# PlanNoa/video_super_resolution

Measured on NVIDIA B200. Metric: sr_frames_per_s_4x_1080p_out, higher is better.
Workload: dtype bf16

## Files before the change

include/vsr_b200.h:

```cpp
#ifndef VSR_B200_H_
#define VSR_B200_H_

#include <stddef.h>
#include <stdint.h>

#ifdef __cplusplus
extern "C" {
#endif

#define VSR_OK 0
#define VSR_ERR_INVALID_ARG 1
#define VSR_ERR_UNSUPPORTED 2
#define VSR_ERR_WORKSPACE 3
#define VSR_ERR_STATE 4
#define VSR_ERR_CUDA_BASE 1000

typedef void* vsr_stream_t;

const char* vsr_version(void);
uint64_t vsr_launch_count(void);
void vsr_launch_count_reset(void);
const char* vsr_error_string(int code);

int vsr_resample2d_forward(const float* input1, const float* flow, float* output,
// ... 156 lines not shown
int vsr_srfbn_profile_launches(vsr_srfbn_plan* plan, float* ms, int32_t* kclass, int32_t capacity);

int vsr_srfbn_debug_premix(const vsr_srfbn_plan* plan, float* out_maps, vsr_stream_t stream);

int vsr_test_pointwise(const void* x_bf16, int64_t rows, int K, const float* w_host,
                       const float* b_host, float slope, int act, void* y_bf16,
                       void* workspace, size_t workspace_bytes, vsr_stream_t stream);
int vsr_test_deconv(const void* x_bf16, int B, int h, int w, const float* w_host,
                    const float* b_host, float slope, int block_layout, void* y_bf16,
                    void* workspace, size_t workspace_bytes, vsr_stream_t stream);
int vsr_test_x2_layer(const void* x_bf16, int up, int B, int h, int w, const float* w_host,
                      const float* b_host, float slope, void* y_bf16, void* workspace,
                      size_t workspace_bytes, vsr_stream_t stream);
size_t vsr_test_workspace_bytes(int B, int h, int w);
int vsr_test_fused_down(const void* hr_bf16, int nsrc, int B, int h, int w, const float* wt_host,
                        const float* bt_host, float slope_t, const float* wd_host, const float* bd_host,
                        float slope_d, void* y_bf16, void* workspace, size_t workspace_bytes,
                        vsr_stream_t stream);
int vsr_test_fused_updown(const void* lr_bf16, void* hr_bf16, int nsrc, int store, int B, int h, int w,
                          const float* wu_host, const float* bu_host, float slope_u, const float* wt_host,
                          const float* bt_host, float slope_t, const float* wd_host, const float* bd_host,
                          float slope_d, void* y_bf16, void* workspace, size_t workspace_bytes,
                          vsr_stream_t stream);

#ifdef __cplusplus
}
#endif
#endif
```

video_super_resolution_b200/_lib.py:

```python
from __future__ import annotations

import ctypes
import os

_HERE = os.path.dirname(os.path.abspath(__file__))
LIB_PATH = os.path.join(_HERE, "libvsr_b200.so")

c_void_p = ctypes.c_void_p
c_int = ctypes.c_int
c_i64 = ctypes.c_int64
c_size_t = ctypes.c_size_t
c_float = ctypes.c_float


class VsrError(RuntimeError):
    pass


class SrfbnConfig(ctypes.Structure):
    _fields_ = [("num_maps", ctypes.c_int32), ("h", ctypes.c_int32), ("w", ctypes.c_int32),
                ("num_steps", ctypes.c_int32), ("num_groups", ctypes.c_int32),
                ("num_features", ctypes.c_int32), ("upscale", ctypes.c_int32)]


# ... 60 lines not shown
    "vsr_srfbn_forward": (c_int, [c_void_p, c_void_p, c_void_p, c_void_p]),
    "vsr_srfbn_forward_u8": (c_int, [c_void_p, c_void_p, c_void_p, c_void_p, c_void_p]),
    "vsr_srfbn_prepare_refresh": (c_int, [c_void_p, c_int]),
    "vsr_srfbn_forward_refresh_u8": (c_int, [c_void_p, c_void_p, c_void_p, c_void_p, c_int, c_void_p]),
    "vsr_srfbn_plan_set_map_range": (c_int, [c_void_p, c_int, c_int]),
    "vsr_srfbn_forward_maps": (c_int, [c_void_p, c_void_p, c_void_p]),
    "vsr_srfbn_forward_maps_refresh": (c_int, [c_void_p, c_void_p, c_int, c_void_p]),
    "vsr_srfbn_pack_bands": (c_int, [c_void_p, ctypes.POINTER(c_int), c_int, c_void_p, c_void_p]),
    "vsr_srfbn_fuse_band": (c_int, [c_void_p, c_void_p, c_int, c_void_p, c_void_p, c_void_p]),
    "vsr_unpack_bands": (c_int, [c_void_p, c_void_p, c_int, c_i64, c_i64, ctypes.POINTER(c_int), c_int, c_i64,
                                 c_void_p]),
    "vsr_srfbn_kernel_class_name":(ctypes.c_char_p, [c_int]),
    "vsr_srfbn_profile_enable": (c_int, [c_void_p, c_int]),
    "vsr_srfbn_profile_read": (c_int, [c_void_p, c_void_p, c_void_p, c_void_p, c_void_p]),
    "vsr_srfbn_profile_launches": (c_int, [c_void_p, c_void_p, c_void_p, c_int]),
    "vsr_srfbn_debug_premix": (c_int, [c_void_p, c_void_p, c_void_p]),
    "vsr_test_pointwise": (c_int, [c_void_p, c_i64, c_int, c_void_p, c_void_p, c_float, c_int, c_void_p, c_void_p, c_size_t, c_void_p]),
    "vsr_test_deconv": (c_int, [c_void_p, c_int, c_int, c_int, c_void_p, c_void_p, c_float, c_int, c_void_p, c_void_p, c_size_t, c_void_p]),
    "vsr_test_fused_down": (c_int, [c_void_p, c_int, c_int, c_int, c_int, c_void_p, c_void_p, c_float, c_void_p, c_void_p,
                                    c_float, c_void_p, c_void_p, c_size_t, c_void_p]),
    "vsr_test_fused_updown": (c_int, [c_void_p, c_void_p, c_int, c_int, c_int, c_int, c_int, c_void_p, c_void_p, c_float,
                                      c_void_p, c_void_p, c_float, c_void_p, c_void_p, c_float, c_void_p, c_void_p,
                                      c_size_t, c_void_p]),
    "vsr_test_x2_layer": (c_int, [c_void_p, c_int, c_int, c_int, c_int, c_void_p, c_void_p, c_float, c_void_p, c_void_p, c_size_t, c_void_p]),
    "vsr_test_workspace_bytes": (c_size_t, [c_int, c_int, c_int]),
}

_lib = None


def lib():
    global _lib
    if _lib is None:
        if not os.path.exists(LIB_PATH):
            raise ImportError(
                f"{LIB_PATH} is missing: build it with `python -m video_super_resolution_b200.build` "
                "(nvcc, sm_100a).  This package has no CPU or PyTorch fallback.")
        L = ctypes.CDLL(LIB_PATH)
        for name, (res, args) in SIGNATURES.items():
            fn = getattr(L, name)
            fn.restype = res
            fn.argtypes = args
        _lib = L
    return _lib


# ... 13 lines not shown
```

video_super_resolution_b200/csrc/fused_down.cuh:

```cuda
#pragma once
#include "igemm.cuh"

namespace vsr {

constexpr int kFusedEpiWarps = 16;
constexpr int kFusedWdWarp = 2 + kFusedEpiWarps;
constexpr int kFusedBWarp = kFusedWdWarp + 1;
constexpr int kFusedThreads = 32 * (kFusedBWarp + 1);
constexpr int kFusedMaxStages = 16;
constexpr int kWdGroupBytes = 128 * 128 * 2;
constexpr int kWdRingBytes = 2 * kWdGroupBytes;
constexpr int kWtChunkBytes = 32 * 32 * 2;
constexpr int kHBytes = 128 * 128 * 2;
constexpr int kXchgBytes = 3 * 4 * 16 * 8 * 4;
constexpr int kLRBox = 16 * 9 * 64;
constexpr int kLRBytes = 2 * kLRBox;
constexpr int kWuTapBytes = 128 * 32 * 2;

struct alignas(64) FusedDownParams {
  CUtensorMap hr_maps[kMaxSources];
  CUtensorMap h0_map;
  CUtensorMap wt_map;
  CUtensorMap wd_map;
  int32_t nsrc;
// ... 4 lines not shown
  const float* down_bias;
  float* part;
  void* lr_out;
  CUtensorMap up_map;
  CUtensorMap wu_map;
  const float* up_bias;
  int32_t hr_store;
};

__device__ __forceinline__ void tmem_ld8(uint32_t taddr, uint32_t (&v)[8]) {
  asm volatile("tcgen05.ld.sync.aligned.32x32b.x8.b32 {%0, %1, %2, %3, %4, %5, %6, %7}, [%8];"
               : "=r"(v[0]), "=r"(v[1]), "=r"(v[2]), "=r"(v[3]), "=r"(v[4]), "=r"(v[5]), "=r"(v[6]), "=r"(v[7])
               : "r"(taddr)
               : "memory");
}

template <bool HAS_TRAN>
inline size_t fused_down_smem_bytes(int nsrc, int num_stages) {
  size_t wt = HAS_TRAN ? ((size_t)nsrc * kWtChunkBytes + 1023) / 1024 * 1024 : 0;
  size_t stage = HAS_TRAN ? 16384 : 2 * 16384;
  return 1024 + kWdRingBytes + wt + (HAS_TRAN ? kHBytes : 0) + (size_t)num_stages * stage + 1024 + kXchgBytes;
}

inline size_t fused_updown_smem_bytes(int nsrc, int num_stages) {
  return fused_down_smem_bytes<true>(nsrc, num_stages) + kLRBytes;
}

template <bool HAS_TRAN, bool MERGED>
__device__ __forceinline__ void fused_down_body(const FusedDownParams& p) {
  static_assert(HAS_TRAN || !MERGED, "the merged kernel needs phase A");
  constexpr int kStageBytes = HAS_TRAN ? 16384 : 2 * 16384;
  constexpr int kTmemCols = HAS_TRAN ? 512 : 256;
  constexpr uint32_t kDB = MERGED ? 384 : HAS_TRAN ? 256 : 0;
  constexpr int kDBToggle = MERGED ? 0 : 1;
  constexpr uint32_t kTU = 256;

  extern __shared__ uint8_t smem_raw[];
  uint8_t* smem = smem_raw + ((1024u - (smem_u32(smem_raw) & 1023u)) & 1023u);
  uint8_t* s_wd = smem;
  uint8_t* s_wt = s_wd + kWdRingBytes;
  const int wt_region = HAS_TRAN ? ((p.nsrc * kWtChunkBytes + 1023) / 1024 * 1024) : 0;
  uint8_t* s_h = s_wt + wt_region;
  uint8_t* s_lr = s_h + (HAS_TRAN ? kHBytes : 0);
  uint8_t* s_a = s_lr + (MERGED ? kLRBytes : 0);
  uint8_t* tail = s_a + p.num_stages * kStageBytes;
  uint64_t* full_bar = reinterpret_cast<uint64_t*>(tail);
  uint64_t* empty_bar = full_bar + kFusedMaxStages;
  uint64_t* w_full = empty_bar + kFusedMaxStages;
  uint64_t* wd_full = w_full + 1;
  uint64_t* wd_empty = wd_full + 2;
  uint64_t* da_full = wd_empty + 2;
  uint64_t* da_empty = da_full + 2;
  uint64_t* h_full = da_empty + 2;
  uint64_t* h_empty = h_full + 1;
  uint64_t* db_full = h_empty + 1;
  uint64_t* db_empty = db_full + 2;
  uint32_t* tmem_ptr = reinterpret_cast<uint32_t*>(db_empty + 2);
  uint64_t* tu_full = db_empty + 3;
  uint64_t* tu_empty = tu_full + 1;
  uint64_t* u_full = tu_empty + 1;
  uint64_t* lr_full = u_full + 1;
  uint64_t* lr_empty = lr_full + 1;
  float* s_bias = reinterpret_cast<float*>(tail + 512);
  float* s_down = s_bias + 36;
  float* s_ubias = s_down + 36;
  float4* s_x = reinterpret_cast<float4*>(tail + 1024);
// ... 80 lines not shown
                tma_load_4d(s_a + s * kStageBytes + 16384, &p.h0_map, &full_bar[s], 0, x0, y0, b * 8 + 2 * g + 1);
              }
              __syncwarp();
              if (++s == p.num_stages) { s = 0; phase ^= 1; }
            }
          }
        }
      }
    }
  } else if (warp == 1 || (HAS_TRAN && warp == kFusedBWarp)) {
    {
    constexpr uint32_t idesc_a = make_idesc(32);
    constexpr uint32_t idesc_b = make_idesc(128);
    if (HAS_TRAN && warp == 1) mbar_wait(w_full, 0);
    tc_fence_after();
    int s = 0;
    uint32_t phase = 0;
    uint32_t n_a[2] = {0, 0}, n_b[2] = {0, 0}, n_h = 0, n_wd = 0;
    int tb = 0;
    const uint64_t dA = make_smem_desc<128>(smem_u32(s_a));
    const uint64_t dWt = make_smem_desc<64>(smem_u32(s_wt));
    const uint64_t dH = make_smem_desc<128>(smem_u32(s_h));
    const uint64_t dWd = make_smem_desc<128>(smem_u32(s_wd));
    uint32_t n_tu = 0, n_lr = 0, n_u = 0;

    auto issue_u = [&](int g) {
      constexpr uint32_t idesc_u = make_idesc(128);
      const uint64_t dLR = make_smem_desc<64>(smem_u32(s_lr));
      const uint64_t dWu = make_smem_desc<64>(smem_u32(s_wd));
      if (g == 0) mbar_wait(lr_full, n_lr & 1);
      mbar_wait(tu_empty, (n_tu & 1) ^ 1);
      mbar_wait(&wd_full[0], n_tu & 1);
      tc_fence_after();
      if (elect_one()) {
#pragma unroll
        for (int t = 0; t < 4; ++t)
#pragma unroll
          for (int k = 0; k < 2; ++k)
            umma_bf16(tmem_base + kTU, dLR + (uint64_t)(((t & 1) * kLRBox + (t >> 1) * 1024) >> 4) + 2 * k,
                      dWu + (uint64_t)((t * kWuTapBytes) >> 4) + 2 * k, idesc_u, (uint32_t)((t | k) != 0));
        umma_commit(&wd_empty[0]);
        umma_commit(tu_full);
        if (g == 3) umma_commit(lr_empty);
      }
      __syncwarp();
      ++n_tu;
      if (g == 3) ++n_lr;
    };

    auto issue_a = [&](int g) {
      const int buf = g & 1;
      mbar_wait(&da_empty[buf], (n_a[buf] & 1) ^ 1);
      tc_fence_after();
      for (int pair = 0; pair < 2; ++pair)
        for (int j = 0; j < p.nsrc - (MERGED ? 1 : 0); ++j) {
          mbar_wait(&full_bar[s], phase);
          tc_fence_after();
          const uint64_t a0 = dA + (uint64_t)((s * kStageBytes) >> 4);
          const uint64_t b0 = dWt + (uint64_t)((j * kWtChunkBytes) >> 4);
          const uint32_t d0 = tmem_base + (uint32_t)(buf * 128 + pair * 64);
          if (elect_one()) {
            const uint32_t acc = (uint32_t)(j != 0);
            umma_bf16(d0, a0, b0, idesc_a, acc);
            umma_bf16(d0, a0 + 2, b0 + 2, idesc_a, 1u);
            umma_bf16(d0 + 32, a0 + 4, b0, idesc_a, acc);
            umma_bf16(d0 + 32, a0 + 6, b0 + 2, idesc_a, 1u);
            umma_commit(&empty_bar[s]);
            if (!MERGED && pair == 1 && j == p.nsrc - 1) umma_commit(&da_full[buf]);
          }
          __syncwarp();
          if (++s == p.num_stages) { s = 0; phase ^= 1; }
        }
      if (MERGED) {
        mbar_wait(u_full, n_u & 1);
        tc_fence_after();
        const uint64_t b0 = dWt + (uint64_t)(((p.nsrc - 1) * kWtChunkBytes) >> 4);
        if (elect_one()) {
          for (int pair = 0; pair < 2; ++pair) {
            const uint64_t a0 = dH + (uint64_t)((pair * 16384) >> 4);
            const uint32_t d0 = tmem_base + (uint32_t)(buf * 128 + pair * 64);
            umma_bf16(d0, a0, b0, idesc_a, 1u);
            umma_bf16(d0, a0 + 2, b0 + 2, idesc_a, 1u);
            umma_bf16(d0 + 32, a0 + 4, b0, idesc_a, 1u);
            umma_bf16(d0 + 32, a0 + 6, b0 + 2, idesc_a, 1u);
          }
          umma_commit(&da_full[buf]);
        }
        __syncwarp();
        ++n_u;
      }
      ++n_a[buf];
    };
    auto issue_b = [&](int g) {
      uint64_t a0;
      if (HAS_TRAN) {
        mbar_wait(h_full, n_h & 1);
        a0 = dH;
      } else {
        mbar_wait(&full_bar[s], phase);
        a0 = dA + (uint64_t)((s * kStageBytes) >> 4);
      }
      if (g == 0) mbar_wait(&db_empty[tb], (n_b[tb] & 1) ^ 1);
      const int wslot = MERGED ? 1 : (int)(n_wd & 1);
      mbar_wait(&wd_full[wslot], MERGED ? (n_wd & 1) : ((n_wd >> 1) & 1));
      tc_fence_after();
      const uint32_t d = tmem_base + kDB + (uint32_t)(tb * 128);
      const uint64_t b0 = dWd + (uint64_t)((wslot * kWdGroupBytes) >> 4);
      if (elect_one()) {
#pragma unroll
        for (int kc = 0; kc < 2; ++kc)
#pragma unroll
          for (int k = 0; k < 4; ++k)
            umma_bf16(d, a0 + (uint64_t)(kc * 1024 + k * 2), b0 + (uint64_t)(kc * 1024 + k * 2), idesc_b,
                      (uint32_t)((g | kc | k) != 0));
        umma_commit(&wd_empty[wslot]);
        if (HAS_TRAN) umma_commit(h_empty);
        else umma_commit(&empty_bar[s]);
        if (g == 3) umma_commit(&db_full[tb]);
      }
      __syncwarp();
      ++n_wd;
      if (HAS_TRAN) ++n_h;
      else if (++s == p.num_stages) { s = 0; phase ^= 1; }
      if (g == 3) { ++n_b[tb]; tb ^= kDBToggle; }
    };

    for (int tile = cta; tile < total_tiles; tile += ncta) {
      if (HAS_TRAN) {
        if (warp == 1) {
          for (int g = 0; g < 4; ++g) {
            if (MERGED) issue_u(g);
            issue_a(g);
          }
        } else {
          for (int g = 0; g < 4; ++g) issue_b(g);
        }
      } else {
        for (int g = 0; g < 4; ++g) issue_b(g);
      }
    }
    }
  } else if (MERGED && warp == kFusedWdWarp) {
    uint32_t n_wu = 0, n_wdm = 0, n_lrl = 0;
    auto load_u = [&](int tile, int g) {
      if (g == 0) {
        int x0, y0, b;
        tile_coord(tile, x0, y0, b);
        mbar_wait(lr_empty, (n_lrl & 1) ^ 1);
        if (elect_one()) {
          mbar_expect_tx(lr_full, (uint32_t)kLRBytes);
          tma_load_4d(s_lr, &p.up_map, lr_full, 0, x0 - 1, y0 - 1, b);
          tma_load_4d(s_lr + kLRBox, &p.up_map, lr_full, 0, x0, y0 - 1, b);
        }
        __syncwarp();
        ++n_lrl;
// ... 48 lines not shown
      tile_coord(tile, x0, y0, b);
      const int Yb = y0 + (row >> 4), Xb = x0 + (row & 15);
      const bool in_tensor = (Yb <= p.lr_h) && (Xb <= p.lr_w);
      if (HAS_TRAN) {
#pragma unroll 1
        for (int g = 0; g < 4; ++g) {
          const int buf = g & 1;
          if (MERGED) {
            mbar_wait_poll(tu_full, m_u & 1);
            tc_fence_after();
            uint32_t v[32];
            tmem_ld32(lane_base + kTU + (uint32_t)(sub * 32), v);
            tmem_ld_wait();
            tc_fence_before();
            mbar_arrive_warp(tu_empty);
            ++m_u;
            const int s16 = g * 4 + sub, ry = s16 >> 2, rx = s16 & 3;
            const int Yt = 4 * Yb + ry - 2, Xt = 4 * Xb + rx - 2;
            const bool inside = (Yt >= 0) && (Yt < 4 * p.lr_h) && (Xt >= 0) && (Xt < 4 * p.lr_w);
            uint32_t o[16];
            const PreluCfg pcu = make_prelu(s_ubias[32], 1);
            convert32(v, s_ubias, pcu, o);
            if (__builtin_expect(!inside, 0)) zero16(o);
            mbar_wait(h_empty, (m_h & 1) ^ 1);
            uint8_t* urow = s_h + (sub >> 1) * 16384 + row * 128;
#pragma unroll
            for (int j = 0; j < 4; ++j) {
              const int piece = (sub & 1) * 4 + j;
              *reinterpret_cast<uint4*>(urow + ((piece ^ (row & 7)) << 4)) =
                  make_uint4(o[4 * j], o[4 * j + 1], o[4 * j + 2], o[4 * j + 3]);
            }
            fence_async_smem();
            asm volatile("bar.sync 1, %0;" ::"n"(32 * kFusedEpiWarps) : "memory");
            if (threadIdx.x == 64) {
              if (p.hr_store) {
                tma_store_4d(&p.hr_maps[p.nsrc - 1], s_h, 0, x0, y0, b * 8 + 2 * g);
                tma_store_4d(&p.hr_maps[p.nsrc - 1], s_h + 16384, 0, x0, y0, b * 8 + 2 * g + 1);
                tma_store_commit();
              }
              mbar_arrive(u_full);
            }
          }
          mbar_wait_poll(&da_full[buf], m_a[buf] & 1);
          tc_fence_after();
          uint32_t o[16];
          uint32_t v[32];
          tmem_ld32(lane_base + (uint32_t)(buf * 128 + sub * 32), v);
          tmem_ld_wait();
          tc_fence_before();
          mbar_arrive_warp(&da_empty[buf]);
          const int s16 = g * 4 + sub, ry = s16 >> 2, rx = s16 & 3;
          const bool ring = (Yb == 0 && ry < 2) || (Yb == p.lr_h && ry >= 2) || (Xb == 0 && rx < 2) ||
                            (Xb == p.lr_w && rx >= 2);
          convert32(v, s_bias, pc, o);
          if (__builtin_expect(!(in_tensor && !ring), 0)) zero16(o);
          ++m_a[buf];
          if (MERGED) {
            if (p.hr_store) {
              if (threadIdx.x == 64) tma_store_wait_read();
              asm volatile("bar.sync 1, %0;" ::"n"(32 * kFusedEpiWarps) : "memory");
            }
          } else {
            mbar_wait(h_empty, (m_h & 1) ^ 1);
          }
          uint8_t* hrow = s_h + (sub >> 1) * 16384 + (row >> 3) * 1024 + (row & 7) * 128;
#pragma unroll
          for (int j = 0; j < 4; ++j) {
            const int piece = (sub & 1) * 4 + j;
            *reinterpret_cast<uint4*>(hrow + ((piece ^ (row & 7)) << 4)) =
                make_uint4(o[4 * j], o[4 * j + 1], o[4 * j + 2], o[4 * j + 3]);
          }
          fence_async_smem();
          mbar_arrive_warp(h_full);
          ++m_h;
        }
      }
      mbar_wait_poll(&db_full[tb], m_b[tb] & 1);
      tc_fence_after();
      uint32_t v[4][8];
#pragma unroll
// ... 56 lines not shown
          }
        }
      }
      ++m_b[tb];
      tb ^= kDBToggle;
    }
    if (MERGED && threadIdx.x == 64) asm volatile("cp.async.bulk.wait_group 0;" ::: "memory");
  }

  tc_fence_before();
  __syncthreads();
  if (warp == 1) {
    tc_fence_after();
    tmem_dealloc<kTmemCols>(tmem_base);
  }
}

template <bool HAS_TRAN>
__global__ void __launch_bounds__(kFusedThreads, 1)
fused_down_kernel(const __grid_constant__ FusedDownParams p) {
  fused_down_body<HAS_TRAN, false>(p);
}

__global__ void __launch_bounds__(kFusedThreads, 1)
fused_updown_kernel(const __grid_constant__ FusedDownParams p) {
  fused_down_body<true, true>(p);
}

constexpr int kFinalizePeriod = 8;
__global__ void __launch_bounds__(256)
finalize_lr_kernel(const float4* __restrict__ part, const float* __restrict__ bias, uint4* __restrict__ out, int B, int h,
                   int w) {
  constexpr int period = kFinalizePeriod;
  const float slope = __ldg(bias + 32);
  const int R = h / period, Cc = w / 16;
  const int64_t nA = (int64_t)B * R * w, nB = (int64_t)B * (h - R) * Cc;
  const int64_t n8 = (nA + nB) * 4;
  for (int64_t i = (int64_t)blockIdx.x * blockDim.x + threadIdx.x; i < n8; i += (int64_t)gridDim.x * blockDim.x) {
    const int c8 = (int)(i & 3);
    int64_t it = i >> 2;
    int b, Y, X;
    if (it < nA) {
      X = (int)(it % w);
      const int64_t r = it / w;
      Y = (int)(r % R) * period + period - 1;
      b = (int)(r / R);
    } else {
      it -= nA;
      X = (int)(it % Cc) * 16 + 15;
// ... 26 lines not shown
```

video_super_resolution_b200/csrc/srfbn.cu:

```cuda
#include "fused_down.cuh"

#include <string.h>

#include <algorithm>
#include <new>
#include <vector>

namespace vsr {
namespace {

constexpr int kNF = 32;
constexpr int kGroups = 6;
constexpr int kMaxMaps = 64;

typedef CUresult (*EncodeTiledFn)(CUtensorMap*, CUtensorMapDataType, cuuint32_t, void*, const cuuint64_t*,
                                  const cuuint64_t*, const cuuint32_t*, const cuuint32_t*, CUtensorMapInterleave,
                                  CUtensorMapSwizzle, CUtensorMapL2promotion, CUtensorMapFloatOOBfill);

EncodeTiledFn encode_fn() {
  static EncodeTiledFn fn = nullptr;
  if (!fn) {
    void* p = nullptr;
    cudaDriverEntryPointQueryResult q;
    if (cudaGetDriverEntryPoint("cuTensorMapEncodeTiled", &p, cudaEnableDefault, &q) == cudaSuccess &&
// ... 9 lines not shown
  cuuint64_t dims[4] = {(cuuint64_t)C, (cuuint64_t)W, (cuuint64_t)H, (cuuint64_t)B};
  cuuint64_t strides[3] = {(cuuint64_t)C * 2, (cuuint64_t)C * 2 * W, (cuuint64_t)C * 2 * W * H};
  cuuint32_t box[4] = {(cuuint32_t)ck, (cuuint32_t)tw, (cuuint32_t)th, 1};
  cuuint32_t es[4] = {1, 1, 1, 1};
  CUresult r = enc(m, CU_TENSOR_MAP_DATA_TYPE_BFLOAT16, 4, const_cast<void*>(base), dims, strides, box, es,
                   CU_TENSOR_MAP_INTERLEAVE_NONE, ck == 32 ? CU_TENSOR_MAP_SWIZZLE_64B : CU_TENSOR_MAP_SWIZZLE_128B,
                   CU_TENSOR_MAP_L2_PROMOTION_L2_128B, CU_TENSOR_MAP_FLOAT_OOB_FILL_NONE);
  return r == CUDA_SUCCESS ? VSR_OK : VSR_ERR_CUDA_BASE + 999;
}

int make_w_map(CUtensorMap* m, const void* base, int64_t K, int64_t N, int ck, int bn) {
  EncodeTiledFn enc = encode_fn();
  if (!enc) return VSR_ERR_STATE;
  cuuint64_t dims[2] = {(cuuint64_t)K, (cuuint64_t)N};
  cuuint64_t strides[1] = {(cuuint64_t)K * 2};
  cuuint32_t box[2] = {(cuuint32_t)ck, (cuuint32_t)bn};
  cuuint32_t es[2] = {1, 1};
  CUresult r = enc(m, CU_TENSOR_MAP_DATA_TYPE_BFLOAT16, 2, const_cast<void*>(base), dims, strides, box, es,
                   CU_TENSOR_MAP_INTERLEAVE_NONE, ck == 32 ? CU_TENSOR_MAP_SWIZZLE_64B : CU_TENSOR_MAP_SWIZZLE_128B,
                   CU_TENSOR_MAP_L2_PROMOTION_L2_256B, CU_TENSOR_MAP_FLOAT_OOB_FILL_NONE);
  return r == CUDA_SUCCESS ? VSR_OK : VSR_ERR_CUDA_BASE + 999;
}

enum Variant : int { V_PW32 = 0, V_PW128, V_DECONV, V_CONVOUT, V_FUSED_TRAN, V_FUSED_PLAIN, V_FINALIZE, V_DECONV2, V_DOWN2, V_FUSED_UPDOWN, V_COUNT };

static_assert(VSR_SRFBN_KERNEL_CLASSES == 10, "header constant");
enum KClass : int { KC_IM2COL = 0, KC_CONV_IN, KC_PW_LR, KC_PW_HR, KC_DECONV, KC_DOWNCONV, KC_CONV_OUT, KC_FC, KC_FUSED_DOWN, KC_FINALIZE, KC_COUNT };

struct Layer {
  int variant;
  IgemmParams p;
  FusedDownParams f;
  float* fin_acc;
  const float* fin_bias;
  void* fin_out;
  int64_t fin_n8;
  int fin_w, fin_h, fin_b;
  int grid;
  size_t smem;
  int kclass;
  double flops;
  double bytes;
};

template <int MODE, int CK, int BN>
int launch_variant(const Layer& L, cudaStream_t st) {
  static PerDeviceOnce once;
// ... 2 lines not shown
    cudaError_t e = cudaFuncSetAttribute(igemm_kernel<MODE, CK, BN>, cudaFuncAttributeMaxDynamicSharedMemorySize,
                                         227 * 1024);
    if (e != cudaSuccess) return cuda_status(e);
    once.mark(dev);
  }
  igemm_kernel<MODE, CK, BN><<<L.grid, igemm_threads(MODE), L.smem, st>>>(L.p);
  return after_launch();
}

template <bool HAS_TRAN>
int launch_fused(const Layer& L, cudaStream_t st) {
  static PerDeviceOnce once;
  int dev;
  if (once.needed(&dev)) {
    cudaError_t e = cudaFuncSetAttribute(fused_down_kernel<HAS_TRAN>, cudaFuncAttributeMaxDynamicSharedMemorySize,
                                         227 * 1024);
    if (e != cudaSuccess) return cuda_status(e);
    once.mark(dev);
  }
  fused_down_kernel<HAS_TRAN><<<L.grid, kFusedThreads, L.smem, st>>>(L.f);
  return after_launch();
}

int launch_fused_updown(const Layer& L, cudaStream_t st) {
  static PerDeviceOnce once;
  int dev;
  if (once.needed(&dev)) {
    cudaError_t e = cudaFuncSetAttribute(fused_updown_kernel, cudaFuncAttributeMaxDynamicSharedMemorySize, 227 * 1024);
    if (e != cudaSuccess) return cuda_status(e);
    once.mark(dev);
  }
  fused_updown_kernel<<<L.grid, kFusedThreads, L.smem, st>>>(L.f);
  return after_launch();
}

int launch_layer(const Layer& L, cudaStream_t st) {
  switch (L.variant) {
    case V_FUSED_UPDOWN: return launch_fused_updown(L, st);
    case V_FUSED_TRAN: return launch_fused<true>(L, st);
    case V_FUSED_PLAIN: return launch_fused<false>(L, st);
    case V_FINALIZE: {
      const int R = L.fin_h / kFinalizePeriod;
      const int64_t items = ((int64_t)L.fin_b * R * L.fin_w + (int64_t)L.fin_b * (L.fin_h - R) * (L.fin_w / 16)) * 4;
      if (items == 0) return VSR_OK;
      int64_t blocks = ceil_div64(items, 256);
      if (blocks > kNumSMs * 16) blocks = kNumSMs * 16;
      finalize_lr_kernel<<<(int)blocks, 256, 0, st>>>(reinterpret_cast<const float4*>(L.fin_acc), L.fin_bias,
                                                      reinterpret_cast<uint4*>(L.fin_out), L.fin_b, L.fin_h, L.fin_w);
      return after_launch();
    }
    case V_PW32: return launch_variant<EPI_ROWS, 32, 32>(L, st);
    case V_PW128: return launch_variant<EPI_ROWS, 32, 128>(L, st);
    case V_DECONV: return launch_variant<EPI_DECONV, 32, 256>(L, st);
    case V_CONVOUT: return launch_variant<EPI_CONV_OUT, 32, 32>(L, st);
    case V_DECONV2: return launch_variant<EPI_DECONV2, 32, 128>(L, st);
    case V_DOWN2: return launch_variant<EPI_DOWN2, 64, 96>(L, st);
    default: return VSR_ERR_INVALID_ARG;
  }
}

size_t variant_smem(int variant, int chunks, size_t ring) {
// ... 278 lines not shown
  f.num_stages = tran ? 7 : 5;
  f.tiles_x = ceil_div(w + 1, 16);
  f.tiles_y = ceil_div(h + 1, 8);
  f.batch = B;
  f.lr_h = h;
  f.lr_w = w;
  f.tran_bias = tran_bias_dev;
  f.down_bias = down_bias_dev;
  f.part = part;
  f.lr_out = lr_out;
  while (f.num_stages > 2 && (tran ? fused_down_smem_bytes<true>(nsrc, f.num_stages)
                                   : fused_down_smem_bytes<false>(nsrc, f.num_stages)) > 227 * 1024)
    --f.num_stages;
  L.smem = tran ? fused_down_smem_bytes<true>(nsrc, f.num_stages) : fused_down_smem_bytes<false>(nsrc, f.num_stages);
  int64_t total = (int64_t)f.tiles_x * f.tiles_y * B;
  L.grid = (int)(total < kNumSMs ? total : kNumSMs);
  const double lrpx = (double)B * h * w;
  L.kclass = KC_FUSED_DOWN;
  L.flops = lrpx * 131072.0 + (tran ? lrpx * 16.0 * 2.0 * 32.0 * nsrc * 32.0 : 0.0);
  L.bytes = lrpx * 64.0 * (16.0 * nsrc) + lrpx * 64.0;
  return VSR_OK;
}

inline bool updown_merged(int nsrc) { return nsrc >= 4; }

int build_fused_updown(Layer& L, const void* up_in, const void* const* hr, int nsrc, int store, int B, int h, int w,
                       const void* wu_dev, const float* up_bias_dev, const void* wt_dev, const float* tran_bias_dev,
                       const void* wd_dev, const float* down_bias_dev, float* part, void* lr_out) {
  memset(&L, 0, sizeof(L));
  L.variant = V_FUSED_UPDOWN;
  FusedDownParams& f = L.f;
  if (nsrc < 2 || nsrc > kMaxSources || (store && !hr[nsrc - 1])) return VSR_ERR_UNSUPPORTED;
  int rc;
  for (int j = 0; j < nsrc - (store ? 0 : 1); ++j) {
    rc = make_act_map(&f.hr_maps[j], hr[j], 64, w + 1, h + 1, 8 * B, 64, 16, 8);
    if (rc) return rc;
  }
  rc = make_w_map(&f.wt_map, wt_dev, 32 * nsrc, 32, 32, 32);
  if (rc) return rc;
  rc = make_w_map(&f.wd_map, wd_dev, 512, 128, 64, 128);
  if (rc) return rc;
  rc = make_act_map(&f.up_map, up_in, kNF, w, h, B, 32, kTW, kTH + 1);
  if (rc) return rc;
  rc = make_w_map(&f.wu_map, wu_dev, 4 * kNF, 512, 32, 128);
  if (rc) return rc;
  f.nsrc = nsrc;
  f.tiles_x = ceil_div(w + 1, 16);
  f.tiles_y = ceil_div(h + 1, 8);
  f.batch = B;
  f.lr_h = h;
  f.lr_w = w;
  f.tran_bias = tran_bias_dev;
  f.down_bias = down_bias_dev;
  f.up_bias = up_bias_dev;
  f.part = part;
  f.lr_out = lr_out;
  f.hr_store = store;
  const int64_t total = (int64_t)f.tiles_x * f.tiles_y * B;
  L.grid = (int)(total < kNumSMs ? total : kNumSMs);
  f.num_stages = 7;
  while (f.num_stages > 2 && fused_updown_smem_bytes(nsrc, f.num_stages) > 227 * 1024) --f.num_stages;
  L.smem = fused_updown_smem_bytes(nsrc, f.num_stages);
  const double lrpx = (double)B * h * w;
  L.kclass = KC_FUSED_DOWN;
  L.flops = lrpx * 131072.0 * 2.0 + lrpx * 16.0 * 2.0 * 32.0 * nsrc * 32.0;
  L.bytes = lrpx * 64.0 + lrpx * 64.0 * 16.0 * (nsrc - 1 + (store ? 1 : 0)) + lrpx * 64.0;
  return VSR_OK;
}

int build_finalize(Layer& L, float* acc, const float* bias_dev, void* out, int64_t pixels, int h, int w) {
  memset(&L, 0, sizeof(L));
  L.variant = V_FINALIZE;
  L.fin_acc = acc;
  L.fin_bias = bias_dev;
  L.fin_out = out;
  L.fin_n8 = pixels * 4;
  L.fin_w = w;
  L.fin_h = h;
  L.fin_b = (int)(pixels / ((int64_t)h * w));
  L.kclass = KC_FINALIZE;
  L.flops = 0;
  L.bytes = 0;
  return VSR_OK;
}

// ... 299 lines not shown

static int swept_maps(const vsr_srfbn_plan* pl) { return pl->windows * (pl->map1 - pl->map0); }

static bool all_maps(const vsr_srfbn_plan* pl) { return pl->map1 - pl->map0 == pl->cfg.num_maps; }

static void layout_workspace(vsr_srfbn_plan* pl, int chunk, int swept) {
  const vsr_srfbn_config& c = pl->cfg;
  const size_t P = (size_t)chunk * c.h * c.w;
  const size_t Rb = (size_t)chunk * (c.h + 1) * (c.w + 1) * 16;
  size_t off = 0;
  auto put = [&](size_t bytes) {
    size_t o = off;
    off = align_up(off + bytes, 1024);
    return o;
  };
  pl->o_a0 = put(P * 64);
  pl->o_c128 = put(P * 256);
  pl->o_xfeat = put(P * 64);
  pl->o_hidden = put(P * 64);
  for (int i = 0; i < 7; ++i) pl->o_lr[i] = put(P * 64);
  pl->o_u = put(P * 64);
  const size_t s2 = (size_t)c.upscale * c.upscale;
  const bool x2 = c.upscale == 2;
  for (int i = 0; i < 6; ++i) pl->o_hr[i] = put(x2 ? P * s2 * 64 : (i == 5 && updown_merged(6)) ? 0 : Rb * 64);
  pl->o_hb = put(P * s2 * 64);
  pl->o_ht = put(x2 ? P * s2 * 64 : 0);
  pl->o_acc = put(x2 ? 0 : P * 512);
  pl->o_premix = put((size_t)swept * c.h * c.w * s2 * 3 * 4);
  pl->ws_bytes = off;
}

static int set_shape(vsr_srfbn_plan* pl, int windows, int m0, int m1) {
  if (windows > 1 && m1 - m0 != pl->cfg.num_maps) return VSR_ERR_UNSUPPORTED;
  const int swept = windows * (m1 - m0);
  for (int mc = swept; mc >= 1; --mc) {
    if (swept % mc) continue;
    layout_workspace(pl, mc, swept);
    if (pl->ws_cap == 0 || pl->ws_bytes <= pl->ws_cap) {
      pl->windows = windows;
      pl->map0 = m0;
      pl->map1 = m1;
      pl->chunk_maps = mc;
      return VSR_OK;
    }
  }
  layout_workspace(pl, pl->chunk_maps, swept_maps(pl));
  return VSR_ERR_WORKSPACE;
// ... 173 lines not shown
      if (i > 0) {
        Src s[6];
        for (int j = 0; j <= i; ++j) s[j] = Src{ws + pl->o_lr[j], 32, 0, 32};
        PUSH(build_pointwise(L, s, i + 1, P, Wp(W_UPTRAN0 + i - 1), Bp(W_UPTRAN0 + i - 1), 32, 1, ws + pl->o_u, 64, 0,
                             0, h, w));
        up_in = ws + pl->o_u;
      }
      if (c.upscale == 2) {
        PUSH(build_deconv2(L, up_in, M, h, w, Wp(W_UP0 + i), Bp(W_UP0 + i), ws + pl->o_hr[i]));
        const void* down_in = ws + pl->o_hr[0];
        if (i > 0) {
          Src s[6];
          for (int j = 0; j <= i; ++j) s[j] = Src{ws + pl->o_hr[j], 32, 0, 32};
          rc = build_pointwise(L, s, i + 1, P * 4, Wp(W_DOWNTRAN0 + i - 1), Bp(W_DOWNTRAN0 + i - 1), 32, 1,
                               ws + pl->o_ht, 64, 0, 0, h, w);
          if (rc) return rc;
          L.kclass = KC_PW_HR;
          layers.push_back(L);
          down_in = ws + pl->o_ht;
        }
        PUSH(build_downconv2(L, down_in, M, h, w, Wp(W_DOWN0 + i), Bp(W_DOWN0 + i), ws + pl->o_lr[i + 1]));
        continue;
      }
      if (updown_merged(i + 1)) {
        const void* hrs[6];
        for (int j = 0; j <= i; ++j) hrs[j] = ws + pl->o_hr[j];
        const int store = i + 1 < kGroups;
        if (!store) hrs[i] = nullptr;
        PUSH(build_fused_updown(L, up_in, hrs, i + 1, store, M, h, w, Wp(W_UP0 + i), Bp(W_UP0 + i),
                                Wp(W_DOWNTRAN0 + i - 1), Bp(W_DOWNTRAN0 + i - 1), Wp(W_DOWN0 + i), Bp(W_DOWN0 + i),
                                reinterpret_cast<float*>(ws + pl->o_acc), ws + pl->o_lr[i + 1]));
        PUSH(build_finalize(L, reinterpret_cast<float*>(ws + pl->o_acc), Bp(W_DOWN0 + i), ws + pl->o_lr[i + 1], P, h, w));
      } else {
        Layer D, F;
        rc = build_deconv(D, up_in, M, h, w, Wp(W_UP0 + i), Bp(W_UP0 + i), ws + pl->o_hr[i], 0);
        if (rc) return rc;
        const void* hrs[6];
        for (int j = 0; j <= i; ++j) hrs[j] = ws + pl->o_hr[j];
        rc = build_fused_down(F, hrs, i + 1, M, h, w, i > 0 ? Wp(W_DOWNTRAN0 + i - 1) : nullptr,
                              i > 0 ? Bp(W_DOWNTRAN0 + i - 1) : nullptr, Wp(W_DOWN0 + i), Bp(W_DOWN0 + i),
                              reinterpret_cast<float*>(ws + pl->o_acc), ws + pl->o_lr[i + 1]);
        if (rc) return rc;
        layers.push_back(D);
        layers.push_back(F);
        PUSH(build_finalize(L, reinterpret_cast<float*>(ws + pl->o_acc), Bp(W_DOWN0 + i), ws + pl->o_lr[i + 1], P, h, w));
      }
    }
    {
      Src s[6];
      for (int j = 0; j < 6; ++j) s[j] = Src{ws + pl->o_lr[j + 1], 32, 0, 32};
      PUSH(build_pointwise(L, s, 6, P, Wp(W_COMPRESS_OUT), Bp(W_COMPRESS_OUT), 32, 1, ws + pl->o_hidden, 64, 0, 0, h,
                           w));
// ... 396 lines not shown
    if (rc) return rc;
    memcpy(bt, bt_host, 32 * 4);
    bt[32] = slope_t;
    rc = upload(ws + 257 * 1024, bt, sizeof(bt), st);
    if (rc) return rc;
  }
  float* acc = reinterpret_cast<float*>(ws + base_bytes);
  const void* hrs[6];
  const size_t plane = (size_t)B * (h + 1) * (w + 1) * 16 * 64;
  for (int j = 0; j < nsrc; ++j) hrs[j] = reinterpret_cast<const uint8_t*>(hr_bf16) + j * plane;
  Layer L;
  rc = build_fused_down(L, hrs, nsrc, B, h, w, ws + 160 * 1024, reinterpret_cast<const float*>(ws + 257 * 1024), ws,
                        reinterpret_cast<const float*>(ws + 256 * 1024), acc, y_bf16);
  if (rc) return rc;
  rc = launch_layer(L, st);
  if (rc) return rc;
  rc = build_finalize(L, acc, reinterpret_cast<const float*>(ws + 256 * 1024), y_bf16, (int64_t)B * h * w, h, w);
  if (rc) return rc;
  rc = launch_layer(L, st);
  if (rc) return rc;
  return cuda_status(cudaStreamSynchronize(st));
}

extern "C" int vsr_test_fused_updown(const void* lr_bf16, void* hr_bf16, int nsrc, int store, int B, int h, int w,
                                     const float* wu_host, const float* bu_host, float slope_u, const float* wt_host,
                                     const float* bt_host, float slope_t, const float* wd_host, const float* bd_host,
                                     float slope_d, void* y_bf16, void* workspace, size_t workspace_bytes,
                                     vsr_stream_t stream) {
  if (!lr_bf16 || !hr_bf16 || !wu_host || !bu_host || !wt_host || !bt_host || !wd_host || !bd_host || !y_bf16 ||
      !workspace || B <= 0 || h <= 0 || w <= 0 || nsrc < 2 || nsrc > 6)
    return VSR_ERR_INVALID_ARG;
  const size_t base_bytes = vsr_test_workspace_bytes(B, h, w);
  const size_t acc_bytes = (size_t)B * h * w * 512;
  if (workspace_bytes < base_bytes + acc_bytes) return VSR_ERR_WORKSPACE;
  cudaStream_t st = as_stream(stream);
  uint8_t* ws = reinterpret_cast<uint8_t*>(workspace);
  std::vector<uint16_t> wd((size_t)128 * 512), wu((size_t)512 * 128), wt((size_t)32 * 32 * nsrc);
  pack_downconv_fused(wd_host, wd.data());
  pack_deconv(wu_host, wu.data());
  pack_pointwise(wt_host, 32, 32 * nsrc, wt.data());
  float bd[33], bt[33], bu[33];
  memcpy(bd, bd_host, 32 * 4);
  bd[32] = slope_d;
  memcpy(bt, bt_host, 32 * 4);
  bt[32] = slope_t;
  memcpy(bu, bu_host, 32 * 4);
  bu[32] = slope_u;
  int rc = upload(ws, wd.data(), wd.size() * 2, st);
  if (!rc) rc = upload(ws + 160 * 1024, wt.data(), wt.size() * 2, st);
  if (!rc) rc = upload(ws + 384 * 1024, wu.data(), wu.size() * 2, st);
  if (!rc) rc = upload(ws + 256 * 1024, bd, sizeof(bd), st);
  if (!rc) rc = upload(ws + 257 * 1024, bt, sizeof(bt), st);
  if (!rc) rc = upload(ws + 258 * 1024, bu, sizeof(bu), st);
  if (rc) return rc;
  float* acc = reinterpret_cast<float*>(ws + base_bytes);
  const void* hrs[6];
  const size_t plane = (size_t)B * (h + 1) * (w + 1) * 16 * 64;
  for (int j = 0; j < nsrc; ++j) hrs[j] = reinterpret_cast<const uint8_t*>(hr_bf16) + j * plane;
  if (!store) hrs[nsrc - 1] = nullptr;
  const float* bd_dev = reinterpret_cast<const float*>(ws + 256 * 1024);
  const float* bt_dev = reinterpret_cast<const float*>(ws + 257 * 1024);
  const float* bu_dev = reinterpret_cast<const float*>(ws + 258 * 1024);
  Layer L;
  rc = build_fused_updown(L, lr_bf16, hrs, nsrc, store, B, h, w, ws + 384 * 1024, bu_dev, ws + 160 * 1024, bt_dev, ws,
                          bd_dev, acc, y_bf16);
  if (rc) return rc;
  rc = launch_layer(L, st);
  if (rc) return rc;
  rc = build_finalize(L, acc, bd_dev, y_bf16, (int64_t)B * h * w, h, w);
  if (rc) return rc;
  rc = launch_layer(L, st);
  if (rc) return rc;
  return cuda_status(cudaStreamSynchronize(st));
}
```

Baseline: 11.02.

## Add split-buffer fused up/down kernel and merge layers for groups 2-4

```diff
diff --git a/include/vsr_b200.h b/include/vsr_b200.h
--- a/include/vsr_b200.h
+++ b/include/vsr_b200.h
@@ -202,6 +202,11 @@
                           const float* bt_host, float slope_t, const float* wd_host, const float* bd_host,
                           float slope_d, void* y_bf16, void* workspace, size_t workspace_bytes,
                           vsr_stream_t stream);
+int vsr_test_fused_updown_form(const void* lr_bf16, void* hr_bf16, int nsrc, int store, int B, int h, int w,
+                               const float* wu_host, const float* bu_host, float slope_u, const float* wt_host,
+                               const float* bt_host, float slope_t, const float* wd_host, const float* bd_host,
+                               float slope_d, void* y_bf16, void* workspace, size_t workspace_bytes,
+                               vsr_stream_t stream, int form);
 
 #ifdef __cplusplus
 }
diff --git a/video_super_resolution_b200/_lib.py b/video_super_resolution_b200/_lib.py
--- a/video_super_resolution_b200/_lib.py
+++ b/video_super_resolution_b200/_lib.py
@@ -106,6 +106,9 @@
     "vsr_test_fused_updown": (c_int, [c_void_p, c_void_p, c_int, c_int, c_int, c_int, c_int, c_void_p, c_void_p, c_float,
                                       c_void_p, c_void_p, c_float, c_void_p, c_void_p, c_float, c_void_p, c_void_p,
                                       c_size_t, c_void_p]),
+    "vsr_test_fused_updown_form": (c_int, [c_void_p, c_void_p, c_int, c_int, c_int, c_int, c_int, c_void_p, c_void_p,
+                                           c_float, c_void_p, c_void_p, c_float, c_void_p, c_void_p, c_float, c_void_p,
+                                           c_void_p, c_size_t, c_void_p, c_int]),
     "vsr_test_x2_layer": (c_int, [c_void_p, c_int, c_int, c_int, c_int, c_void_p, c_void_p, c_float, c_void_p, c_void_p, c_size_t, c_void_p]),
     "vsr_test_workspace_bytes": (c_size_t, [c_int, c_int, c_int]),
 }
diff --git a/video_super_resolution_b200/csrc/fused_down.cuh b/video_super_resolution_b200/csrc/fused_down.cuh
--- a/video_super_resolution_b200/csrc/fused_down.cuh
+++ b/video_super_resolution_b200/csrc/fused_down.cuh
@@ -50,13 +50,14 @@
   return 1024 + kWdRingBytes + wt + (HAS_TRAN ? kHBytes : 0) + (size_t)num_stages * stage + 1024 + kXchgBytes;
 }
 
-inline size_t fused_updown_smem_bytes(int nsrc, int num_stages) {
-  return fused_down_smem_bytes<true>(nsrc, num_stages) + kLRBytes;
-}
-
-template <bool HAS_TRAN, bool MERGED>
+inline size_t fused_updown_smem_bytes(int nsrc, int num_stages, bool split) {
+  return fused_down_smem_bytes<true>(nsrc, num_stages) + kLRBytes + (split ? kHBytes : 0);
+}
+
+template <bool HAS_TRAN, bool MERGED, bool SPLIT = false>
 __device__ __forceinline__ void fused_down_body(const FusedDownParams& p) {
   static_assert(HAS_TRAN || !MERGED, "the merged kernel needs phase A");
+  static_assert(MERGED || !SPLIT, "only the merged kernel has a U buffer");
   constexpr int kStageBytes = HAS_TRAN ? 16384 : 2 * 16384;
   constexpr int kTmemCols = HAS_TRAN ? 512 : 256;
   constexpr uint32_t kDB = MERGED ? 384 : HAS_TRAN ? 256 : 0;
@@ -69,7 +70,8 @@
   uint8_t* s_wt = s_wd + kWdRingBytes;
   const int wt_region = HAS_TRAN ? ((p.nsrc * kWtChunkBytes + 1023) / 1024 * 1024) : 0;
   uint8_t* s_h = s_wt + wt_region;
-  uint8_t* s_lr = s_h + (HAS_TRAN ? kHBytes : 0);
+  uint8_t* s_u = SPLIT ? s_h + kHBytes : s_h;
+  uint8_t* s_lr = s_h + (HAS_TRAN ? kHBytes : 0) + (SPLIT ? kHBytes : 0);
   uint8_t* s_a = s_lr + (MERGED ? kLRBytes : 0);
   uint8_t* tail = s_a + p.num_stages * kStageBytes;
   uint64_t* full_bar = reinterpret_cast<uint64_t*>(tail);
@@ -196,6 +198,7 @@
     const uint64_t dWt = make_smem_desc<64>(smem_u32(s_wt));
     const uint64_t dH = make_smem_desc<128>(smem_u32(s_h));
     const uint64_t dWd = make_smem_desc<128>(smem_u32(s_wd));
+    const uint64_t dU = make_smem_desc<128>(smem_u32(s_u));
     uint32_t n_tu = 0, n_lr = 0, n_u = 0;
 
     auto issue_u = [&](int g) {
@@ -222,7 +225,7 @@
       if (g == 3) ++n_lr;
     };
 
-    auto issue_a = [&](int g) {
+    auto issue_a_ring = [&](int g) {
       const int buf = g & 1;
       mbar_wait(&da_empty[buf], (n_a[buf] & 1) ^ 1);
       tc_fence_after();
@@ -245,24 +248,26 @@
           __syncwarp();
           if (++s == p.num_stages) { s = 0; phase ^= 1; }
         }
-      if (MERGED) {
-        mbar_wait(u_full, n_u & 1);
-        tc_fence_after();
-        const uint64_t b0 = dWt + (uint64_t)(((p.nsrc - 1) * kWtChunkBytes) >> 4);
-        if (elect_one()) {
-          for (int pair = 0; pair < 2; ++pair) {
-            const uint64_t a0 = dH + (uint64_t)((pair * 16384) >> 4);
-            const uint32_t d0 = tmem_base + (uint32_t)(buf * 128 + pair * 64);
-            umma_bf16(d0, a0, b0, idesc_a, 1u);
-            umma_bf16(d0, a0 + 2, b0 + 2, idesc_a, 1u);
-            umma_bf16(d0 + 32, a0 + 4, b0, idesc_a, 1u);
-            umma_bf16(d0 + 32, a0 + 6, b0 + 2, idesc_a, 1u);
-          }
-          umma_commit(&da_full[buf]);
-        }
-        __syncwarp();
-        ++n_u;
-      }
+      if (!MERGED) ++n_a[buf];
+    };
+    auto issue_a_u = [&](int g) {
+      const int buf = g & 1;
+      mbar_wait(u_full, n_u & 1);
+      tc_fence_after();
+      const uint64_t b0 = dWt + (uint64_t)(((p.nsrc - 1) * kWtChunkBytes) >> 4);
+      if (elect_one()) {
+        for (int pair = 0; pair < 2; ++pair) {
+          const uint64_t a0 = dU + (uint64_t)((pair * 16384) >> 4);
+          const uint32_t d0 = tmem_base + (uint32_t)(buf * 128 + pair * 64);
+          umma_bf16(d0, a0, b0, idesc_a, 1u);
+          umma_bf16(d0, a0 + 2, b0 + 2, idesc_a, 1u);
+          umma_bf16(d0 + 32, a0 + 4, b0, idesc_a, 1u);
+          umma_bf16(d0 + 32, a0 + 6, b0 + 2, idesc_a, 1u);
+        }
+        umma_commit(&da_full[buf]);
+      }
+      __syncwarp();
+      ++n_u;
       ++n_a[buf];
     };
     auto issue_b = [&](int g) {
@@ -302,9 +307,12 @@
     for (int tile = cta; tile < total_tiles; tile += ncta) {
       if (HAS_TRAN) {
         if (warp == 1) {
+          if (SPLIT) issue_u(0);
           for (int g = 0; g < 4; ++g) {
-            if (MERGED) issue_u(g);
-            issue_a(g);
+            if (MERGED && !SPLIT) issue_u(g);
+            issue_a_ring(g);
+            if (SPLIT && g < 3) issue_u(g + 1);
+            if (MERGED) issue_a_u(g);
           }
         } else {
           for (int g = 0; g < 4; ++g) issue_b(g);
@@ -399,8 +407,15 @@
             const PreluCfg pcu = make_prelu(s_ubias[32], 1);
             convert32(v, s_ubias, pcu, o);
             if (__builtin_expect(!inside, 0)) zero16(o);
-            mbar_wait(h_empty, (m_h & 1) ^ 1);
-            uint8_t* urow = s_h + (sub >> 1) * 16384 + row * 128;
+            if (SPLIT) {
+              if (p.hr_store) {
+                if (threadIdx.x == 64) tma_store_wait_read();
+                asm volatile("bar.sync 1, %0;" ::"n"(32 * kFusedEpiWarps) : "memory");
+              }
+            } else {
+              mbar_wait(h_empty, (m_h & 1) ^ 1);
+            }
+            uint8_t* urow = s_u + (sub >> 1) * 16384 + row * 128;
 #pragma unroll
             for (int j = 0; j < 4; ++j) {
               const int piece = (sub & 1) * 4 + j;
@@ -411,8 +426,8 @@
             asm volatile("bar.sync 1, %0;" ::"n"(32 * kFusedEpiWarps) : "memory");
             if (threadIdx.x == 64) {
               if (p.hr_store) {
-                tma_store_4d(&p.hr_maps[p.nsrc - 1], s_h, 0, x0, y0, b * 8 + 2 * g);
-                tma_store_4d(&p.hr_maps[p.nsrc - 1], s_h + 16384, 0, x0, y0, b * 8 + 2 * g + 1);
+                tma_store_4d(&p.hr_maps[p.nsrc - 1], s_u, 0, x0, y0, b * 8 + 2 * g);
+                tma_store_4d(&p.hr_maps[p.nsrc - 1], s_u + 16384, 0, x0, y0, b * 8 + 2 * g + 1);
                 tma_store_commit();
               }
               mbar_arrive(u_full);
@@ -432,7 +447,7 @@
           convert32(v, s_bias, pc, o);
           if (__builtin_expect(!(in_tensor && !ring), 0)) zero16(o);
           ++m_a[buf];
-          if (MERGED) {
+          if (MERGED && !SPLIT) {
             if (p.hr_store) {
               if (threadIdx.x == 64) tma_store_wait_read();
               asm volatile("bar.sync 1, %0;" ::"n"(32 * kFusedEpiWarps) : "memory");
@@ -535,9 +550,10 @@
   fused_down_body<HAS_TRAN, false>(p);
 }
 
+template <bool SPLIT>
 __global__ void __launch_bounds__(kFusedThreads, 1)
 fused_updown_kernel(const __grid_constant__ FusedDownParams p) {
-  fused_down_body<true, true>(p);
+  fused_down_body<true, true, SPLIT>(p);
 }
 
 constexpr int kFinalizePeriod = 8;
diff --git a/video_super_resolution_b200/csrc/srfbn.cu b/video_super_resolution_b200/csrc/srfbn.cu
--- a/video_super_resolution_b200/csrc/srfbn.cu
+++ b/video_super_resolution_b200/csrc/srfbn.cu
@@ -55,7 +55,7 @@
   return r == CUDA_SUCCESS ? VSR_OK : VSR_ERR_CUDA_BASE + 999;
 }
 
-enum Variant : int { V_PW32 = 0, V_PW128, V_DECONV, V_CONVOUT, V_FUSED_TRAN, V_FUSED_PLAIN, V_FINALIZE, V_DECONV2, V_DOWN2, V_FUSED_UPDOWN, V_COUNT };
+enum Variant : int { V_PW32 = 0, V_PW128, V_DECONV, V_CONVOUT, V_FUSED_TRAN, V_FUSED_PLAIN, V_FINALIZE, V_DECONV2, V_DOWN2, V_FUSED_UPDOWN, V_FUSED_UPDOWN_SPLIT, V_COUNT };
 
 static_assert(VSR_SRFBN_KERNEL_CLASSES == 10, "header constant");
 enum KClass : int { KC_IM2COL = 0, KC_CONV_IN, KC_PW_LR, KC_PW_HR, KC_DECONV, KC_DOWNCONV, KC_CONV_OUT, KC_FC, KC_FUSED_DOWN, KC_FINALIZE, KC_COUNT };
@@ -104,21 +104,24 @@
   return after_launch();
 }
 
+template <bool SPLIT>
 int launch_fused_updown(const Layer& L, cudaStream_t st) {
   static PerDeviceOnce once;
   int dev;
   if (once.needed(&dev)) {
-    cudaError_t e = cudaFuncSetAttribute(fused_updown_kernel, cudaFuncAttributeMaxDynamicSharedMemorySize, 227 * 1024);
+    cudaError_t e = cudaFuncSetAttribute(fused_updown_kernel<SPLIT>, cudaFuncAttributeMaxDynamicSharedMemorySize,
+                                         227 * 1024);
     if (e != cudaSuccess) return cuda_status(e);
     once.mark(dev);
   }
-  fused_updown_kernel<<<L.grid, kFusedThreads, L.smem, st>>>(L.f);
+  fused_updown_kernel<SPLIT><<<L.grid, kFusedThreads, L.smem, st>>>(L.f);
   return after_launch();
 }
 
 int launch_layer(const Layer& L, cudaStream_t st) {
   switch (L.variant) {
-    case V_FUSED_UPDOWN: return launch_fused_updown(L, st);
+    case V_FUSED_UPDOWN: return launch_fused_updown<false>(L, st);
+    case V_FUSED_UPDOWN_SPLIT: return launch_fused_updown<true>(L, st);
     case V_FUSED_TRAN: return launch_fused<true>(L, st);
     case V_FUSED_PLAIN: return launch_fused<false>(L, st);
     case V_FINALIZE: {
@@ -443,13 +446,21 @@
   return VSR_OK;
 }
 
-inline bool updown_merged(int nsrc) { return nsrc >= 4; }
-
-int build_fused_updown(Layer& L, const void* up_in, const void* const* hr, int nsrc, int store, int B, int h, int w,
-                       const void* wu_dev, const float* up_bias_dev, const void* wt_dev, const float* tran_bias_dev,
-                       const void* wd_dev, const float* down_bias_dev, float* part, void* lr_out) {
+enum UpdownForm : int { UD_LAYERED = 0, UD_MERGED_SHARED = 1, UD_MERGED_SPLIT = 2 };
+inline UpdownForm updown_form(int nsrc) {
+  constexpr UpdownForm kForm[kMaxSources + 1] = {UD_LAYERED, UD_LAYERED, UD_MERGED_SPLIT, UD_MERGED_SPLIT,
+                                                 UD_MERGED_SPLIT, UD_MERGED_SHARED, UD_MERGED_SHARED};
+  return kForm[nsrc];
+}
+
+int build_fused_updown(Layer& L, UpdownForm form, const void* up_in, const void* const* hr, int nsrc, int store, int B,
+                       int h, int w, const void* wu_dev, const float* up_bias_dev, const void* wt_dev,
+                       const float* tran_bias_dev, const void* wd_dev, const float* down_bias_dev, float* part,
+                       void* lr_out) {
   memset(&L, 0, sizeof(L));
-  L.variant = V_FUSED_UPDOWN;
+  if (form != UD_MERGED_SHARED && form != UD_MERGED_SPLIT) return VSR_ERR_UNSUPPORTED;
+  const bool split = form == UD_MERGED_SPLIT;
+  L.variant = split ? V_FUSED_UPDOWN_SPLIT : V_FUSED_UPDOWN;
   FusedDownParams& f = L.f;
   if (nsrc < 2 || nsrc > kMaxSources || (store && !hr[nsrc - 1])) return VSR_ERR_UNSUPPORTED;
   int rc;
@@ -480,8 +491,8 @@
   const int64_t total = (int64_t)f.tiles_x * f.tiles_y * B;
   L.grid = (int)(total < kNumSMs ? total : kNumSMs);
   f.num_stages = 7;
-  while (f.num_stages > 2 && fused_updown_smem_bytes(nsrc, f.num_stages) > 227 * 1024) --f.num_stages;
-  L.smem = fused_updown_smem_bytes(nsrc, f.num_stages);
+  while (f.num_stages > 2 && fused_updown_smem_bytes(nsrc, f.num_stages, split) > 227 * 1024) --f.num_stages;
+  L.smem = fused_updown_smem_bytes(nsrc, f.num_stages, split);
   const double lrpx = (double)B * h * w;
   L.kclass = KC_FUSED_DOWN;
   L.flops = lrpx * 131072.0 * 2.0 + lrpx * 16.0 * 2.0 * 32.0 * nsrc * 32.0;
@@ -827,7 +838,7 @@
   pl->o_u = put(P * 64);
   const size_t s2 = (size_t)c.upscale * c.upscale;
   const bool x2 = c.upscale == 2;
-  for (int i = 0; i < 6; ++i) pl->o_hr[i] = put(x2 ? P * s2 * 64 : (i == 5 && updown_merged(6)) ? 0 : Rb * 64);
+  for (int i = 0; i < 6; ++i) pl->o_hr[i] = put(x2 ? P * s2 * 64 : (i == 5 && updown_form(6) != UD_LAYERED) ? 0 : Rb * 64);
   pl->o_hb = put(P * s2 * 64);
   pl->o_ht = put(x2 ? P * s2 * 64 : 0);
   pl->o_acc = put(x2 ? 0 : P * 512);
@@ -1047,12 +1058,12 @@
         PUSH(build_downconv2(L, down_in, M, h, w, Wp(W_DOWN0 + i), Bp(W_DOWN0 + i), ws + pl->o_lr[i + 1]));
         continue;
       }
-      if (updown_merged(i + 1)) {
+      if (updown_form(i + 1) != UD_LAYERED) {
         const void* hrs[6];
         for (int j = 0; j <= i; ++j) hrs[j] = ws + pl->o_hr[j];
         const int store = i + 1 < kGroups;
         if (!store) hrs[i] = nullptr;
-        PUSH(build_fused_updown(L, up_in, hrs, i + 1, store, M, h, w, Wp(W_UP0 + i), Bp(W_UP0 + i),
+        PUSH(build_fused_updown(L, updown_form(i + 1), up_in, hrs, i + 1, store, M, h, w, Wp(W_UP0 + i), Bp(W_UP0 + i),
                                 Wp(W_DOWNTRAN0 + i - 1), Bp(W_DOWNTRAN0 + i - 1), Wp(W_DOWN0 + i), Bp(W_DOWN0 + i),
                                 reinterpret_cast<float*>(ws + pl->o_acc), ws + pl->o_lr[i + 1]));
         PUSH(build_finalize(L, reinterpret_cast<float*>(ws + pl->o_acc), Bp(W_DOWN0 + i), ws + pl->o_lr[i + 1], P, h, w));
@@ -1495,11 +1506,11 @@
   return cuda_status(cudaStreamSynchronize(st));
 }
 
-extern "C" int vsr_test_fused_updown(const void* lr_bf16, void* hr_bf16, int nsrc, int store, int B, int h, int w,
-                                     const float* wu_host, const float* bu_host, float slope_u, const float* wt_host,
-                                     const float* bt_host, float slope_t, const float* wd_host, const float* bd_host,
-                                     float slope_d, void* y_bf16, void* workspace, size_t workspace_bytes,
-                                     vsr_stream_t stream) {
+static int test_fused_updown(const void* lr_bf16, void* hr_bf16, int nsrc, int store, int B, int h, int w,
+                             const float* wu_host, const float* bu_host, float slope_u, const float* wt_host,
+                             const float* bt_host, float slope_t, const float* wd_host, const float* bd_host,
+                             float slope_d, void* y_bf16, void* workspace, size_t workspace_bytes, vsr_stream_t stream,
+                             UpdownForm form) {
   if (!lr_bf16 || !hr_bf16 || !wu_host || !bu_host || !wt_host || !bt_host || !wd_host || !bd_host || !y_bf16 ||
       !workspace || B <= 0 || h <= 0 || w <= 0 || nsrc < 2 || nsrc > 6)
     return VSR_ERR_INVALID_ARG;
@@ -1535,8 +1546,8 @@
   const float* bt_dev = reinterpret_cast<const float*>(ws + 257 * 1024);
   const float* bu_dev = reinterpret_cast<const float*>(ws + 258 * 1024);
   Layer L;
-  rc = build_fused_updown(L, lr_bf16, hrs, nsrc, store, B, h, w, ws + 384 * 1024, bu_dev, ws + 160 * 1024, bt_dev, ws,
-                          bd_dev, acc, y_bf16);
+  rc = build_fused_updown(L, form, lr_bf16, hrs, nsrc, store, B, h, w, ws + 384 * 1024, bu_dev, ws + 160 * 1024, bt_dev,
+                          ws, bd_dev, acc, y_bf16);
   if (rc) return rc;
   rc = launch_layer(L, st);
   if (rc) return rc;
@@ -1546,3 +1557,23 @@
   if (rc) return rc;
   return cuda_status(cudaStreamSynchronize(st));
 }
+
+extern "C" int vsr_test_fused_updown(const void* lr_bf16, void* hr_bf16, int nsrc, int store, int B, int h, int w,
+                                     const float* wu_host, const float* bu_host, float slope_u, const float* wt_host,
+                                     const float* bt_host, float slope_t, const float* wd_host, const float* bd_host,
+                                     float slope_d, void* y_bf16, void* workspace, size_t workspace_bytes,
+                                     vsr_stream_t stream) {
+  const UpdownForm form = updown_form(nsrc) == UD_MERGED_SHARED ? UD_MERGED_SHARED : UD_MERGED_SPLIT;
+  return test_fused_updown(lr_bf16, hr_bf16, nsrc, store, B, h, w, wu_host, bu_host, slope_u, wt_host, bt_host, slope_t,
+                           wd_host, bd_host, slope_d, y_bf16, workspace, workspace_bytes, stream, form);
+}
+
+extern "C" int vsr_test_fused_updown_form(const void* lr_bf16, void* hr_bf16, int nsrc, int store, int B, int h, int w,
+                                          const float* wu_host, const float* bu_host, float slope_u,
+                                          const float* wt_host, const float* bt_host, float slope_t,
+                                          const float* wd_host, const float* bd_host, float slope_d, void* y_bf16,
+                                          void* workspace, size_t workspace_bytes, vsr_stream_t stream, int form) {
+  if (form != UD_MERGED_SHARED && form != UD_MERGED_SPLIT) return VSR_ERR_INVALID_ARG;
+  return test_fused_updown(lr_bf16, hr_bf16, nsrc, store, B, h, w, wu_host, bu_host, slope_u, wt_host, bt_host, slope_t,
+                           wd_host, bd_host, slope_d, y_bf16, workspace, workspace_bytes, stream, (UpdownForm)form);
+}
```

Measured after the change: 11.11 (median of 6 runs). No clear change (+0.8%).
